# weiquan/salt

Hardware: AMD Instinct MI355X
Metric: Mreads/s aligned (100 bp SE, GRCh38+snp144) at 1/2/4/8 MI355X vs CPU ref (higher is better)
Workload: dtype u32; 1 GPU; GRCh38-scale synthetic (SURVEY 8d config 3 = BASELINE configs[2]): 3100000000 bp genome in 24 contigs, 14800000 SNPs, k=21, 1000000 x 100 bp SE reads per GPU per step, 8 distinct resident batches rotated, inputs and results resident in HBM; read_len=100, distinct_batches=8, options=default (-s 50 -m 1000, overlap = k), streams_per_gpu=4

## Files before the change

### salt_amd/csrc/salt_align.hip

```cpp
#include "salt_device.h"
#include "salt_kernels.h"

namespace salt {

#define WSYNC() do { __builtin_amdgcn_fence(__ATOMIC_ACQ_REL, "wavefront"); __builtin_amdgcn_wave_barrier(); \
                     __builtin_amdgcn_fence(__ATOMIC_ACQ_REL, "wavefront"); } while (0)

static constexpr int MAXL = SALT_MAX_READ_LEN;
static constexpr int SLOTS = SALT_MAX_SEED_SLOTS;
static constexpr int MAXLOC = SALT_MAX_LOCATE;
static constexpr int LVK = 31;
static_assert(offsetof(salt_result_t, strand) == 4 && offsetof(salt_result_t, mapq) == 7 && offsetof(salt_result_t, b0) == 8 &&
              offsetof(salt_result_t, b1) == 12 && offsetof(salt_result_t, seq_start) == 16 && offsetof(salt_result_t, seq_end) == 18 &&
              offsetof(salt_result_t, n_hits) == 20 && offsetof(salt_result_t, n_cigar) == 22 && offsetof(salt_result_t, skipped) == 23 &&
              offsetof(salt_result_t, hits) == 24 && sizeof(salt_hit_t) == 8, "salt_result_t header layout");
static constexpr int NHIT = 6;
__device__ __forceinline__ uint32_t mapq_quot(uint32_t x, uint32_t b0)
{
    const uint32_t v = 255u * x;
    return b0 == 1u ? v : b0 == 2u ? v / 2u : b0 == 3u ? v / 3u : v / b0;
}
static constexpr uint32_t INF = 255;

__device__ __forceinline__ uint32_t lane_id() { return threadIdx.x & 63u; }

typedef const uint32_t __attribute__((address_space(1))) *gp_u32;
typedef uint32_t u32x4_t __attribute__((ext_vector_type(4)));
typedef const u32x4_t __attribute__((address_space(1))) *gp_u32x4;
__device__ __forceinline__ gp_u32 as_global(const uint32_t *p) { return (gp_u32)p; }
__device__ __forceinline__ gp_u32x4 as_global(const uint4 *p) { return (gp_u32x4)(const void *)p; }

struct PhaseClock {
    unsigned long long *acc; uint64_t t;
    __device__ PhaseClock(unsigned long long *a) : acc(a), t(a ? __builtin_amdgcn_s_memtime() : 0) {}
    __device__ __forceinline__ void stamp(int slot)
    {
        if (!acc) return;
        uint64_t n = __builtin_amdgcn_s_memtime();
        if (lane_id() == 0) acc[slot] += (unsigned long long)(n - t);
        t = n;
    }
    __device__ __forceinline__ void add(int slot, unsigned long long v) { if (acc && lane_id() == 0) acc[slot] += v; }
};

__device__ __forceinline__ uint32_t read_base(const uint8_t *seq, uint32_t L, int strand, uint32_t i)
{
    if (strand == 0) return seq[i];
    uint32_t c = seq[L - 1 - i];
    return c < 4 ? 3 - c : c;
}

__device__ __forceinline__ uint32_t pk_nibbles(uint32_t x)
{
    uint32_t t = x & 0x0F0F0F0Fu;
    t = (t | (t >> 4)) & 0x00FF00FFu;
    return (t | (t >> 8)) & 0xFFFFu;
}

struct PackWords { uint32_t pm[64], tb[32], nm[16]; };

__global__ void __launch_bounds__(256)
k_pack(PackGeom pg, uint32_t n_reads, const uint8_t *__restrict__ seqs, const uint32_t *__restrict__ offs,
       uint32_t *__restrict__ pm, uint32_t *__restrict__ tb)
{
    extern __shared__ uint32_t pk_lds[];
    __shared__ uint32_t so[65];
    const uint32_t tpr = pg.nw32, rpb = 256 / tpr < 64 ? 256 / tpr : 64;
    const uint32_t wpr = pg.nw8 + pg.nw16 + pg.nw32;
    const uint32_t r0 = blockIdx.x * rpb, nr = n_reads - r0 < rpb ? n_reads - r0 : rpb;
    if (threadIdx.x <= nr) so[threadIdx.x] = offs[r0 + threadIdx.x];
    __syncthreads();
    const uint32_t cap = 8 * pg.nw8;
    const uint64_t total_bases = offs[n_reads];
    {
        const uint32_t rr = threadIdx.x / tpr, j = threadIdx.x - rr * tpr;
        if (rr < nr) {
            uint32_t L = so[rr + 1] - so[rr];
            if (L > cap) L = cap;
            const uintptr_t a0 = (uintptr_t)seqs + so[rr] + 32u * j, lo = (uintptr_t)seqs & ~(uintptr_t)3, hi = (uintptr_t)seqs + total_bases;
            const uintptr_t ab = a0 & ~(uintptr_t)3;
            const uint32_t sh = (uint32_t)(a0 & 3u) * 8u;
            uint32_t wv[9];
#pragma unroll
// ... 406 lines not shown
    const uint32_t tot_a = a1 - a0, tot = tot_a + (b1 - b0);
    const int i_top = (int)((uint32_t)sp.l_seed - ix.r_lkt_len) - 1;
    uint32_t n_aux = 0, n_sa = 0, n_text = 0, n_occ_c = 0, n_occ_r = 0;
    Walk w; w.ph = WK_IDLE; w.k = w.l = w.ext = w.p0 = 0; w.i = 0;
    SeedCtx c = seed_ctx_geom(sp, tb, 0, ix.r_lkt_len);
    uint32_t item = 0, cur = 0;
    bool is_r = false;
    const uint4 *qp = qa;
    for (;;) {
        const uint64_t idle = __ballot(w.ph == WK_IDLE);
        if (cur >= tot && idle == ~0ull) break;
        if (cur < tot) {
            const uint32_t t = cur + (uint32_t)__popcll(idle & lt);
            if (w.ph == WK_IDLE && t < tot) {
                const bool in_a = t < tot_a;
                qp = in_a ? qa + (size_t)t * WQ_REC : qb + (size_t)(t - tot_a) * WQ_REC; is_r = (in_a ? la : lb) == 0u; w.ph = WK_REC;
            }
            const uint32_t nx = cur + (uint32_t)__popcll(idle);
            cur = nx < tot ? nx : tot;
        }
        WalkReq q = walk_req_none();
        if (w.ph == WK_REC) { q.pa = qp; q.na = WQ_REC; }
        else if (w.ph != WK_IDLE) q = is_r ? seed_walk_issue<true>(ix, sp, c, w) : seed_walk_issue<false>(ix, sp, c, w);
        const WalkLoads ld = walk_fetch(q);
        bool done = false;
        uint4 row = make_uint4(1, 0, 0, 0);
        if (w.ph == WK_REC) {
            item = ld.a[0].x;
            c = seed_ctx_geom(sp, tb, item, ix.r_lkt_len);
            c.w0 = ld.a[1].x; c.w1 = ld.a[1].y; c.w2 = ld.a[1].z; c.n0 = ld.a[0].w; c.n1 = ld.a[1].w;
            done = is_r ? seed_walk_begin<true>(sp, c, ld.a[0].y, ld.a[0].z, i_top, w, row) : seed_walk_begin<false>(sp, c, ld.a[0].y, ld.a[0].z, i_top, w, row);
        } else if (w.ph != WK_IDLE) {
            done = is_r ? seed_walk_finish<true>(ix, sp, c, w, ld, row, n_occ_r, n_aux) : seed_walk_finish<false>(ix, sp, c, w, ld, row, n_occ_c, n_aux);
        }
        if (done && row.x <= row.y) { if (is_r) { row.w = sai_r_pack(sp.epoch, row.w); sai_r[item] = row; } else sai_c[item] = row; }
        n_sa += (n_aux >> 10) & 2047u; n_text += n_aux >> 21; n_aux = 0;
    }
    if (ctr) {
        for (int o = 32; o > 0; o >>= 1) { n_sa += __shfl_down(n_sa, o); n_text += __shfl_down(n_text, o); n_occ_c += __shfl_down(n_occ_c, o); n_occ_r += __shfl_down(n_occ_r, o); }
        if (lane_id() == 0) {
            atomicAdd(ctr + SALT_CTR_OCC_C, n_occ_c); atomicAdd(ctr + SALT_CTR_OCC_R, n_occ_r);
            atomicAdd(ctr + SALT_CTR_D_COCC_SEED, n_occ_c); atomicAdd(ctr + SALT_CTR_D_ROCC_SEED, n_occ_r);
            atomicAdd(ctr + SALT_CTR_D_SA_SEED, n_sa); atomicAdd(ctr + SALT_CTR_D_TEXT_SEED, n_text);
        }
    }
}

template <int NS> struct SaiListsT { uint32_t sp[2][NS], ep[2][NS], off[2][NS]; };
struct SaiLists { uint32_t *sp[2], *ep[2], *off[2]; };
template <int NS> __device__ __forceinline__ SaiLists sai_ref(SaiListsT<NS> &a) { return SaiLists{ { a.sp[0], a.sp[1] }, { a.ep[0], a.ep[1] }, { a.off[0], a.off[1] } }; }
struct LvTables { short L[LVK][64]; char A[LVK][64]; };
static constexpr int LLV_K = 12;
static constexpr int LLV_TW = 22;
static constexpr int LLV_W = 2 * LLV_K + 3;
static constexpr int LLV_N = 64;
struct LaneLv { uint32_t T[LLV_N * LLV_TW]; uint8_t rows[2][LLV_W][LLV_N]; };
struct LvBytes { uint8_t T[MAXL + 4 + 64]; uint8_t P[MAXL + 64]; };
template <int NS, bool LLV>
struct WaveLdsT {
    static constexpr bool HAS_LLV = LLV;
    static constexpr int N_SLOTS = NS;
    uint32_t pm[2][MAXL / 8];
    union U { SaiListsT<NS> sai; typename std::conditional<LLV, LaneLv, uint32_t>::type llv; LvBytes lvb; } u;
    uint8_t  cand_e[MAXLOC];
    uint32_t loci[MAXLOC];
    uint32_t hit_pos[2][NHIT];
    uint8_t  hit_nd[2][NHIT], hit_gap[2][NHIT];
    uint16_t cig[SALT_MAX_CIGAR_OPS];
    int      n_cig;
    alignas(8) uint8_t cargs[128];
};
typedef WaveLdsT<SLOTS, true> WaveLds;
typedef WaveLdsT<32, false> WaveLdsSmall;
typedef WaveLdsT<1, false> WaveLdsCigar;

struct Sai { uint32_t sp, ep, off; };
__device__ __forceinline__ Sai sai_get(const SaiLists &s, int w, int i) { return Sai{ s.sp[w][i], s.ep[w][i], s.off[w][i] }; }
__device__ __forceinline__ void sai_set(SaiLists &s, int w, int i, Sai v) { s.sp[w][i] = v.sp; s.ep[w][i] = v.ep; s.off[w][i] = v.off; }
__device__ __forceinline__ bool sai_ltv(Sai a, Sai b) { return a.ep - a.sp < b.ep - b.sp; }
__device__ __forceinline__ bool sai_lt(const SaiLists &s, int w, int i, int j) { return sai_ltv(sai_get(s, w, i), sai_get(s, w, j)); }
__device__ __forceinline__ void sai_swap(SaiLists &s, int w, int i, int j) { Sai a = sai_get(s, w, i), b = sai_get(s, w, j); sai_set(s, w, i, b); sai_set(s, w, j, a); }

__device__ void sai_insertsort(SaiLists &s, int w, int lo, int hi)
{
    for (int i = lo + 1; i < hi; ++i)
        for (int j = i; j > lo && sai_lt(s, w, j, j - 1); --j) sai_swap(s, w, j, j - 1);
}

__device__ void sai_combsort(SaiLists &s, int w, int base, int n)
{
    const double shrink = 1.2473309501039786540366528676643;
    int gap = n; bool do_swap;
    do {
        if (gap > 2) { gap = (int)(gap / shrink); if (gap == 9 || gap == 10) gap = 11; }
        do_swap = false;
        for (int i = 0; i < n - gap; ++i)
            if (sai_lt(s, w, base + i + gap, base + i)) { sai_swap(s, w, base + i, base + i + gap); do_swap = true; }
    } while (do_swap || gap > 2);
    if (gap != 1) sai_insertsort(s, w, base, base + n);
}

__device__ __attribute__((noinline)) void sai_introsort(SaiLists &s, int w, int n)
{
    if (n < 1) return;
    if (n == 2) { if (sai_lt(s, w, 1, 0)) sai_swap(s, w, 0, 1); return; }
    int d; for (d = 2; (1 << d) < n; ++d) { }
    d <<= 1;
    int st_l[24], st_r[24], st_d[24], top = 0;
    int lo = 0, hi = n - 1;
// ... 390 lines not shown
            }
        }
    }
}

__device__ __attribute__((noinline)) int lv_wave(const uint8_t *T, int tlen, const uint8_t *P, int plen, int k, LvTables *tab, int &d_fin)
{
    const int lane = (int)lane_id();
    const int d = lane - 31;
    const int ad = d < 0 ? -d : d;
    int Lprev = -2;
    const int end0 = plen < tlen ? plen : tlen;
    if (d == 0) { int i = 0; while (i < end0 && (P[i] & T[i]) != 0) ++i; Lprev = i; }
    const int r0 = __shfl(Lprev, 31);
    if (tab) tab->L[0][lane] = (short)Lprev;
    d_fin = 0;
    if (r0 == end0) return plen > end0 ? plen - end0 : 0;
    if (k > LVK - 1) k = LVK - 1;
    for (int e = 1; e <= k; ++e) {
        int left = __shfl_up(Lprev, 1), right = __shfl_down(Lprev, 1);
        if (lane == 0) left = -2;
        if (lane == 63) right = -2;
        const bool active = ad <= e && ad <= LVK - 1;
        int best = Lprev + 1; char act = 'X';
        if (left > best) { best = left; act = 'D'; }
        if (right + 1 > best) { best = right + 1; act = 'I'; }
        int cur = -2;
        if (active) {
            if (P[best] == T[d + best]) {
                int end = plen < tlen - d ? plen : tlen - d;
                if (best >= end) best = end;
                else { int i = best; while (i < end && (P[i] & T[d + i]) != 0) ++i; best = i; }
            }
            cur = best;
        }
        if (tab) { tab->L[e][lane] = (short)cur; tab->A[e][lane] = act; }
        uint64_t reach = __ballot(active && cur == plen);
        if (reach) {
            if (tab) {
                int rank = d == 0 ? 0 : (d < 0 ? 2 * ad - 1 : 2 * ad);
                int my = (active && cur == plen) ? rank : 1000;
                for (int o = 32; o > 0; o >>= 1) { int t = __shfl_xor(my, o); my = t < my ? t : my; }
                d_fin = my == 0 ? 0 : ((my & 1) ? -((my + 1) >> 1) : (my >> 1));
            }
            return e;
        }
        Lprev = cur;
    }
    return -1;
}

__device__ __attribute__((noinline)) uint32_t lv_lanes(LaneLv &s, const uint32_t *pm, int plen, int tlen, int k, bool active)
{
    const int lane = (int)lane_id() & (LLV_N - 1);
    const uint32_t *T = s.T + lane * LLV_TW;
    const int nwp = (plen + 7) >> 3;
    auto wP = [&](int i) -> uint32_t {
        const int j = i >> 3;
        const uint32_t lo = j < nwp ? pm[j] : 0u, hi = j + 1 < nwp ? pm[j + 1] : 0u;
        return __funnelshift_r(lo, hi, 4u * (uint32_t)(i & 7));
    };
    auto wT = [&](int i) -> uint32_t {
        if (i < 0) return i <= -8 ? 0u : T[0] << (4 * -i);
        const int j = i >> 3;
        const uint32_t lo = j < LLV_TW ? T[j] : 0u, hi = j + 1 < LLV_TW ? T[j + 1] : 0u;
        return __funnelshift_r(lo, hi, 4u * (uint32_t)(i & 7));
    };
    auto extend = [&](int d, int i, int end) -> int {
        while (i < end) {
            const uint32_t y = wP(i) & wT(d + i);
            const uint32_t z = ~(((y & 0x77777777u) + 0x77777777u) | y) & 0x88888888u;
            const int run = z ? (__ffs((int)z) - 1) >> 2 : 8;
            i += run;
            if (run < 8) break;
        }
        return i < end ? i : end;
    };
    auto RD = [&](int row, int d) -> int { return (int)s.rows[row][d + LLV_K + 1][lane] - 2; };
    auto WR = [&](int row, int d, int v) { s.rows[row][d + LLV_K + 1][lane] = (uint8_t)(v + 2); };
    for (int row = 0; row < 2; ++row) for (int d = 0; d < LLV_W; ++d) s.rows[row][d][lane] = 0;
    const int end0 = plen < tlen ? plen : tlen;
    uint32_t result = 255;
    bool done = !active;
    if (active) {
        const int i = extend(0, 0, end0);
        WR(0, 0, i);
        if (i == end0) { result = (uint32_t)(plen > end0 ? plen - end0 : 0); done = true; }
    }
    for (int e = 1; e <= k; ++e) {
        if (__ballot(!done) == 0) break;
        const int cur = e & 1, prev = cur ^ 1;
        for (int d = -e; d <= e; ++d) {
            if (done) continue;
            int best = RD(prev, d) + 1;
            const int left = RD(prev, d - 1), right = RD(prev, d + 1) + 1;
            if (left > best) best = left;
            if (right > best) best = right;
            if ((wP(best) & 15u) == (wT(d + best) & 15u)) {
                const int end = plen < tlen - d ? plen : tlen - d;
                best = best >= end ? end : extend(d, best, end);
            }
            if (best == plen) { result = (uint32_t)e; done = true; }
            else WR(cur, d, best);
        }
    }
    return result;
}

template <int VMAX, bool GAPF>
__device__ __forceinline__ void rule_unsorted(const uint32_t *pos, const uint8_t *val, const uint32_t n, const uint32_t L, const uint32_t ref_len,
                                              uint32_t &bound, bool &any, uint32_t &best_pos, uint32_t &best_v,
                                              uint32_t &n_hits, uint32_t &a0, uint32_t *hit_pos, uint8_t *hit_nd)
{
    const uint32_t lane = lane_id();
    const uint32_t NONE = 0xFFFFFFFFu;
    auto in_range = [&](uint32_t p) -> bool { return GAPF ? !(p + L + 4 >= ref_len) : p < ref_len; };
    uint32_t mp[VMAX + 1];
#pragma unroll
    for (int t = 0; t <= VMAX; ++t) mp[t] = NONE;
    uint32_t my_p = 0, my_v = NONE, n_p = 0;
    for (uint32_t b = 0; b < n; b += 64) {
        const uint32_t i = b + lane;
        uint32_t p = 0, v = NONE;
        if (i < n) { p = pos[i]; v = val[i]; }
        const bool in = i < n && v <= bound && in_range(p);
        if (in) {
#pragma unroll
            for (int t = 0; t <= VMAX; ++t) if (v == (uint32_t)t && p < mp[t]) mp[t] = p;
        }
        uint64_t m = __ballot(in);
        if (m && n_p <= 64u) {
            if (n_p + (uint32_t)__popcll(m) > 64u) n_p = 65u;
            else
                while (m) {
                    const int l = __ffsll((long long)m) - 1;
                    const uint32_t pl = (uint32_t)__builtin_amdgcn_readlane((int)p, l), vl = (uint32_t)__builtin_amdgcn_readlane((int)v, l);
                    if (lane == n_p) { my_p = pl; my_v = vl; }
                    ++n_p; m &= m - 1;
                }
        }
    }
#pragma unroll
    for (int t = 0; t <= VMAX; ++t)
        for (int o = 32; o > 0; o >>= 1) { const uint32_t x = (uint32_t)__shfl_xor((int)mp[t], o); mp[t] = x < mp[t] ? x : mp[t]; }
    uint32_t before[VMAX + 1];
    before[0] = NONE;
#pragma unroll
    for (int t = 1; t <= VMAX; ++t) before[t] = mp[t - 1] < before[t - 1] ? mp[t - 1] : before[t - 1];
    any = false; n_hits = 0;
#pragma unroll
    for (int t = VMAX; t >= 0; --t) if (mp[t] != NONE) { any = true; best_v = (uint32_t)t; best_pos = mp[t]; }
    if (!any) return;
    unsigned long long last = 0;
    const bool in_lanes = n_p <= 64u;
    unsigned long long my_key = ~0ull;
    if (in_lanes && lane < n_p) {
// ... 119 lines not shown
        w.u.lvb.P[i] = i < L ? (uint8_t)((w.pm[strand][i >> 3] >> (4 * (i & 7u))) & 15u) : (uint8_t)0;
    }
    WSYNC();
}

template <class W>
__device__ __attribute__((noinline)) void lv_cigar(const uint32_t *ref, W &w, LvTables *tabp, int strand, uint32_t L, uint32_t pos, int k)
{
    LvTables &tab = *tabp;
    lv_unpack(ref, w, strand, L, pos);
    int d_fin = 0;
    WSYNC();
    int e = lv_wave(w.u.lvb.T, (int)L + 4, w.u.lvb.P, (int)L, k, &tab, d_fin);
    __threadfence_block();
    WSYNC();
    if (lane_id() == 0) {
        int n = 0;
        uint16_t *cg = w.cig;
        if (e == 0) { cg[n++] = (uint16_t)((L << 4) | 0u); }
        else if (e > 0) {
            char act[LVK + 1]; int matched[LVK + 1];
            int cd = d_fin;
            for (int ce = e; ce >= 1; --ce) {
                char a = tab.A[ce][cd + 31];
                act[ce] = a;
                int cur = tab.L[ce][cd + 31];
                if (a == 'I') { matched[ce] = cur - tab.L[ce - 1][cd + 1 + 31] - 1; cd += 1; }
                else if (a == 'D') { matched[ce] = cur - tab.L[ce - 1][cd - 1 + 31]; cd -= 1; }
                else { matched[ce] = cur - tab.L[ce - 1][cd + 31] - 1; }
            }
            int acc = tab.L[0][31];
            int ce = 1;
            while (ce <= e) {
                char a = act[ce]; int cnt = 1;
                while (ce + 1 <= e && matched[ce] == 0 && act[ce + 1] == a) { ++cnt; ++ce; }
                if (a == 'X') acc += cnt;
                else {
                    if (acc != 0 && n < SALT_MAX_CIGAR_OPS) { cg[n++] = (uint16_t)((acc << 4) | 0); }
                    acc = 0;
                    if (n < SALT_MAX_CIGAR_OPS) cg[n++] = (uint16_t)((cnt << 4) | (a == 'I' ? 1 : 2));
                }
                if (matched[ce] > 0) acc += matched[ce];
                ++ce;
            }
            if (acc != 0 && n < SALT_MAX_CIGAR_OPS) cg[n++] = (uint16_t)((acc << 4) | 0);
        }
        w.n_cig = n;
    }
    WSYNC();
}

__device__ __forceinline__ void lane_text(const uint32_t *__restrict__ ref, uint32_t *T, uint32_t pos, uint32_t tl)
{
    const uint32_t w0 = pos >> 3, sh = (pos & 7u) * 4u, nwt = (tl + 7) >> 3;
    uint32_t wv[LLV_TW + 1];
#pragma unroll
    for (int j = 0; j <= LLV_TW; ++j) wv[j] = (uint32_t)j <= nwt ? ref[w0 + (uint32_t)j] : 0u;
#pragma unroll
    for (int j = 0; j < LLV_TW; ++j) {
        uint32_t word = 0;
        if ((uint32_t)j < nwt) {
            word = __funnelshift_r(wv[j], wv[j + 1], sh);
            const uint32_t rem = tl - (uint32_t)j * 8;
            if (rem < 8) word &= (1u << (4 * rem)) - 1u;
        }
        T[j] = word;
    }
}

__device__ __forceinline__ uint32_t store_gap_list(const uint32_t *loci, uint32_t n, uint32_t L, uint32_t ref_len, uint32_t *__restrict__ dst)
{
    const uint32_t lane = lane_id();
    const uint64_t lt = (1ull << lane) - 1ull;
    uint32_t n_out = 0;
    for (uint32_t b = 0; b < n; b += 64) {
        const uint32_t i = b + lane;
        const uint32_t pos = i < n ? loci[i] : 0u;
        const bool keep = i < n && !(pos + L + 4 >= ref_len);
        const uint64_t m = __ballot(keep);
        if (keep) dst[n_out + (uint32_t)__popcll(m & lt)] = pos;
        n_out += (uint32_t)__popcll(m);
    }
    return n_out;
}

template <bool PE, bool GL, class W>
__device__ __forceinline__ void align_general(const IndexView ix, const AlignParams ap, W &w, const uint32_t r,
                              const uint32_t *__restrict__ pm,
                              const uint4 *__restrict__ sai_c, const uint4 *__restrict__ sai_r,
                              salt_result_t *__restrict__ results, unsigned long long *__restrict__ ctr,
                              unsigned long long *phase, LvTables *lvtab, const GapBufs g, uint32_t *pe_loci, uint8_t *pe_cand)
{
    const uint32_t lane = lane_id();
    const uint64_t lt = (1ull << lane) - 1ull;
    const uint32_t *rec = pm + (uint64_t)r * ap.pg.pm_stride;
    const uint32_t L = rec[2 * ap.pg.nw8];
    salt_result_t *out = results + r;
    uint32_t c_sa_c = 0, c_sa_r = 0, c_verify = 0, c_vwords = 0, c_lv = 0, c_loci = 0, c_ctx_rej = 0, c_ctx_rows = 0;
    PhaseClock pc(phase);
    const uint64_t rt0 = phase ? __builtin_amdgcn_s_memrealtime() : 0;
    constexpr bool glob = GL;
    uint32_t *loci = glob ? pe_loci : w.loci;
    uint8_t *cand_e = glob ? pe_cand : w.cand_e;
    const uint32_t loci_cap = PE ? PE_LOCI_CAP : (uint32_t)MAXLOC;

    const uint32_t nw = (L + 7) >> 3;
    uint32_t n_amb = 0;
    for (uint32_t t = lane; t < 2 * nw; t += 64) {
        const uint32_t s = t >= nw, j = s ? t - nw : t;
        const uint32_t word = rec[s * ap.pg.nw8 + j];
        w.pm[s][j] = word;
        if (!s) n_amb += (uint32_t)__popc(word & (word >> 1) & (word >> 2) & (word >> 3) & 0x11111111u);
    }
    if (ap.max_amb < L) { for (int o = 32; o > 0; o >>= 1) n_amb += (uint32_t)__shfl_xor((int)n_amb, o); }
    else n_amb = 0;
    WSYNC();
    uint32_t q_pos = 0xFFFFFFFFu; uint32_t q_strand = 3, q_ndiff = 255, q_gap = 255;
    const bool too_short = L < (uint32_t)ap.l_seed;
    if (n_amb > ap.max_amb) {
        if (lane == 0) {
// ... 69 lines not shown
                    uint32_t o = 0;
                    if (lane == 0) o = atomicAdd(&g.gctl->pool_used, n);
                    o = (uint32_t)__shfl((int)o, 0);
                    ok = (uint64_t)o + n <= g.pool;
                    if (ok) for (uint32_t i = lane; i < n; i += 64) g.gloci[o + i] = loci[i];
                    ns[strand] = n; off[strand] = o;
                }
                const uint32_t ch0 = ok ? (ns[0] + LLV_N - 1) / LLV_N : 0, ch1 = ok ? (ns[1] + LLV_N - 1) / LLV_N : 0;
                uint32_t base = 0;
                if (ok && lane == 0) base = atomicAdd(&g.gctl->gap_items, ch0 + ch1);
                base = (uint32_t)__shfl((int)base, 0);
                ok = ok && (uint64_t)base + ch0 + ch1 <= g.items_cap;
                if (lane == 0) {
                    g.gq[slot] = ok ? r : 0xFFFFFFFFu;
                    g.gn[2 * slot] = ok ? ns[0] : 0; g.gn[2 * slot + 1] = ok ? ns[1] : 0;
                    g.goff[2 * slot] = off[0]; g.goff[2 * slot + 1] = off[1];
                }
                if (ok) {
                    for (uint32_t c = lane; c < ch0 + ch1; c += 64) g.gitems[base + c] = (slot << 11) | (c >= ch0 ? (0x400u | (c - ch0)) : c);
                    if (ctr) {
                        for (int o2 = 32; o2 > 0; o2 >>= 1) c_vwords += __shfl_down(c_vwords, o2);
                        if (lane == 0) {
                            atomicAdd(ctr + SALT_CTR_SA_C, c_sa_c); atomicAdd(ctr + SALT_CTR_SA_R, c_sa_r);
                            atomicAdd(ctr + SALT_CTR_VERIFY, c_verify); atomicAdd(ctr + SALT_CTR_VERIFY_WORDS, c_vwords);
                            atomicAdd(ctr + SALT_CTR_LV, ns[0] + ns[1]); atomicAdd(ctr + SALT_CTR_READS, 1ull);
                            atomicAdd(ctr + SALT_CTR_BASES, L); atomicAdd(ctr + SALT_CTR_LOCI, c_loci);
                            atomicAdd(ctr + SALT_CTR_D_SA_HEAVY, c_sa_c + c_sa_r);
                            atomicAdd(ctr + SALT_CTR_D_VERIFY_HEAVY, c_verify * (L <= 248 ? 4u : (((L + 7) >> 3) + 4u) / 4u));
                            atomicAdd(ctr + SALT_CTR_D_OUT_HEAVY, 5u * (ns[0] + ns[1]) + 16u);
                            if (ix.c_ctx) { atomicAdd(ctr + SALT_CTR_D_CTX_ROWS, c_ctx_rows); atomicAdd(ctr + SALT_CTR_D_CTX_REJECTED, c_ctx_rej); }
                        }
                    }
                    return;
                }
                WSYNC();
            }
        }
        if constexpr (!W::HAS_LLV) {
            if (lanes_fit && n_cand_nogap > 0) {
                if (lane == 0) g.ovq[atomicAdd(&g.gctl->ovq_count, 1u)] = r;
                return;
            }
        }
        for (int strand = 0; strand < 2; ++strand) {
            pc.stamp(SALT_CTR_T_GAP);
            const CandStats cs = build_candidates_call<PE, GL>(CandArgs{ ix.c_sa, ix.r_pos, sai_c, sai_r, ix.ref_len, ap.spr, ap.max_locate, r, L, strand, true, phase, pe_loci, loci_cap, ap.pe, true, ap.epoch, nullptr, nullptr, 0 }, w);
            if (glob) { loci = cs.in_lds ? w.loci : pe_loci; cand_e = cs.in_lds ? w.cand_e : pe_cand; }
            pc.t = phase ? __builtin_amdgcn_s_memtime() : 0;
            const uint32_t n_cand = cs.n_cand; c_sa_c += cs.n_sa_c; c_sa_r += cs.n_sa_r; c_loci += cs.n_loci;
            bool any = false;
            const bool lanes_ok = lanes_fit && W::HAS_LLV;
            if constexpr (W::HAS_LLV) if (lanes_ok) {
                const int k0 = gap_k0;
                for (uint32_t b = 0; b < n_cand; b += LLV_N) {
                    WSYNC();
                    const uint32_t i = b + lane;
                    bool act = false;
                    if (lane < LLV_N && i < n_cand) {
                        const uint32_t pos = loci[i];
                        act = !(pos > ix.ref_len || pos + L + 4 > ix.ref_len);
                        if (act) lane_text(ix.ref, w.u.llv.T + lane * LLV_TW, pos, L + 4);
                    }
                    const uint32_t e = lv_lanes(w.u.llv, w.pm[strand], (int)L, (int)L + 4, k0, act);
                    if (lane < LLV_N && i < n_cand) cand_e[i] = (uint8_t)e;
                }
                WSYNC();
            }
            for (uint32_t i = 0; i < n_cand; ++i) {
                uint32_t pos = loci[i];
                int e = -1;
                if (lanes_ok) { const uint32_t ev = cand_e[i]; e = (ev != 255 && (int)ev <= maxd) ? (int)ev : -1; }
                else if (!(pos > ix.ref_len || pos + L + 4 > ix.ref_len)) {
                    lv_unpack(ix.ref, w, strand, L, pos);
                    int dd;
                    e = lv_wave(w.u.lvb.T, (int)L + 4, w.u.lvb.P, (int)L, maxd, nullptr, dd);
                    WSYNC();
                }
                ++c_lv;
                if (e >= 0) {
                    if (e < maxd || !any) { maxd = e; q_gap = 1; q_ndiff = (uint32_t)e; q_strand = (uint32_t)strand; q_pos = pos; }
                    if (n_hits_s[strand] < NHIT && lane == 0) {
                        uint32_t h = n_hits_s[strand];
                        w.hit_pos[strand][h] = pos; w.hit_nd[strand][h] = (uint8_t)e; w.hit_gap[strand][h] = 1;
                    }
                    if (n_hits_s[strand] == 0) a0[strand] = (uint32_t)e;
                    if (n_hits_s[strand] < NHIT) ++n_hits_s[strand];
                    any = true;
                }
            }
            found[strand] = any;
            WSYNC();
        }
    }
    WSYNC();
    pc.stamp(SALT_CTR_T_GAP);

    int b0 = (int)q_ndiff, b1 = 100000, tot = 0;
    uint32_t nh[2] = { 0, 0 };
    uint32_t sel_idx[2][SALT_MAX_HITS];
    for (int s = 0; s < 2 && tot < ap.max_hits; ++s) {
        for (uint32_t j = 0; j < n_hits_s[s]; ++j) {
            uint32_t p = w.hit_pos[s][j];
            if (p == 0xFFFFFFFFu || p == q_pos) continue;
            if (a0[s] <= q_ndiff) {
                if ((int)a0[s] <= b1) b1 = (int)a0[s];
                if (nh[s] < SALT_MAX_HITS) sel_idx[s][nh[s]] = j;
                ++nh[s]; ++tot;
            }
            if (tot == ap.max_hits) break;
        }
    }
    uint32_t mapq = 0;
    if (b0 != 0) {
        uint32_t x = (uint32_t)(b0 > b1 ? b0 - b1 : b1 - b0);
        uint64_t q = mapq_quot(x, (uint32_t)b0);
        mapq = q < 254 ? (uint32_t)q : 254u;
// ... 72 lines not shown
    __shared__ W w;
    __shared__ uint32_t s_item;
    __shared__ unsigned long long s_phase[SALT_CTR_N];
    unsigned long long *phase = ctr ? s_phase : nullptr;
    if (ctr) { for (int i = threadIdx.x; i < SALT_CTR_N; i += 64) s_phase[i] = 0; }
    WSYNC();
    const uint32_t n_items = overflow_pass ? g.gctl->ovq_count : ap.all_heavy ? ap.n_reads : g.gctl->light_queued;
    uint32_t seg = blockIdx.x & (QUEUE_RANGES - 1u), tried = 0;
    for (;;) {
        if (threadIdx.x == 0) {
            uint32_t got = 0xFFFFFFFFu;
            if (overflow_pass) { got = atomicAdd(&g.gctl->ovq_head, 1u); if (got >= n_items) got = 0xFFFFFFFFu; }
            else got = pop_ranged(g.ranges, QueueRange::HEAVY, n_items, seg, tried);
            s_item = got;
        }
        WSYNC();
        const uint32_t it = s_item;
        WSYNC();
        if (it == 0xFFFFFFFFu) break;
        const uint32_t r = overflow_pass ? g.ovq[it] : ap.all_heavy ? it : queue[it];
        align_general<PE, GL>(ix, ap, w, r, pm, sai_c, sai_r, results, ctr, phase, lvtab + blockIdx.x, g,
                          pe_scr ? reinterpret_cast<uint32_t *>(pe_scr + (size_t)blockIdx.x * PE_LOCI_CAP * 5) : nullptr,
                          pe_scr ? pe_scr + (size_t)blockIdx.x * PE_LOCI_CAP * 5 + (size_t)PE_LOCI_CAP * 4 : nullptr);
        if (phase && threadIdx.x == 0) s_phase[SALT_CTR_HEAVY_READS] += 1;
        WSYNC();
    }
    if (phase) {
        WSYNC();
        for (int i = SALT_CTR_T_LOAD + (int)threadIdx.x; i < SALT_CTR_N; i += 64) if (s_phase[i]) atomicAdd(ctr + i, s_phase[i]);
    }
}

#ifndef SALT_HEAVY_WAVES
#define SALT_HEAVY_WAVES 4
#endif
#if SALT_HEAVY_WAVES > 0
#define HEAVY_OCC __attribute__((amdgpu_waves_per_eu(SALT_HEAVY_WAVES, SALT_HEAVY_WAVES)))
#else
#define HEAVY_OCC
#endif
#define HEAVY_KERNEL(NAME, PE, GL, LDS)                                                                                    \
__global__ void __launch_bounds__(64) HEAVY_OCC                                                                         \
NAME(IndexView ix, AlignParams ap, const uint32_t *__restrict__ pm,                                                     \
     const uint4 *__restrict__ sai_c, const uint4 *__restrict__ sai_r, salt_result_t *__restrict__ results,             \
     const uint32_t *__restrict__ queue, unsigned long long *__restrict__ ctr,                                          \
     LvTables *__restrict__ lvtab, GapBufs g, uint8_t *__restrict__ pe_scr, int overflow_pass)                          \
{ heavy_body<PE, GL, LDS>(ix, ap, pm, sai_c, sai_r, results, queue, ctr, lvtab, g, pe_scr, overflow_pass); }
HEAVY_KERNEL(k_heavy, false, false, WaveLdsSmall)
HEAVY_KERNEL(k_heavy_pe, true, true, WaveLdsSmall)
HEAVY_KERNEL(k_heavy_big, false, false, WaveLds)
HEAVY_KERNEL(k_heavy_pe_big, true, true, WaveLds)
HEAVY_KERNEL(k_heavy_glob, false, true, WaveLds)

struct GapLds { LaneLv llv; uint32_t pm[MAXL / 8]; };
__global__ void __launch_bounds__(64)
k_gap(IndexView ix, AlignParams ap, const uint32_t *__restrict__ pm, GapBufs g)
{
    __shared__ GapLds s;
    __shared__ uint32_t s_item;
    const uint32_t lane = lane_id();
    const uint32_t n_items = g.gctl->gap_items < g.items_cap ? g.gctl->gap_items : g.items_cap;
    uint32_t seg = blockIdx.x & (QUEUE_RANGES - 1u), tried = 0;
    for (;;) {
        if (threadIdx.x == 0) s_item = pop_ranged(g.ranges, QueueRange::GAP, n_items, seg, tried);
        WSYNC();
        const uint32_t it = s_item;
        WSYNC();
        if (it == 0xFFFFFFFFu) break;
        const uint32_t item = g.gitems[it], slot = item >> 11, strand = (item >> 10) & 1u, chunk = item & 1023u;
        const uint32_t r = g.gq[slot];
        const uint32_t *rec = pm + (uint64_t)r * ap.pg.pm_stride;
        const uint32_t L = rec[2 * ap.pg.nw8], nw = (L + 7) >> 3;
        for (uint32_t t = lane; t < nw; t += 64) s.pm[t] = rec[strand * ap.pg.nw8 + t];
        const uint32_t n = g.gn[2 * slot + strand], i = chunk * LLV_N + lane;
        const size_t row = g.goff[2 * slot + strand];
        bool act = false;
        if (lane < LLV_N && i < n) {
            const uint32_t pos = g.gloci[row + i];
            act = !(pos > ix.ref_len || pos + L + 4 > ix.ref_len);
            if (act) lane_text(ix.ref, s.llv.T + lane * LLV_TW, pos, L + 4);
        }
        WSYNC();
        const uint32_t e = lv_lanes(s.llv, s.pm, (int)L, (int)L + 4, ap.pe ? 3 : (int)(L / 10), act);
        if (lane < LLV_N && i < n) g.ge[row + i] = (uint8_t)e;
        WSYNC();
    }
}

struct FinLds { uint32_t hit_pos[2][NHIT]; uint8_t hit_nd[2][NHIT]; };
__global__ void __launch_bounds__(64)
k_gapfin(IndexView ix, AlignParams ap, const uint32_t *__restrict__ pm, salt_result_t *__restrict__ results, GapBufs g,
         unsigned long long *__restrict__ ctr)
{
    __shared__ FinLds w;
    __shared__ uint32_t s_item;
    const uint32_t lane = lane_id();
    const uint64_t lt = (1ull << lane) - 1ull;
    const uint32_t n_items = g.gctl->gap_slots < g.cap ? g.gctl->gap_slots : g.cap;
    uint32_t seg = blockIdx.x & (QUEUE_RANGES - 1u), tried = 0;
    for (;;) {
        if (threadIdx.x == 0) s_item = pop_ranged(g.ranges, QueueRange::GAPFIN, n_items, seg, tried);
        WSYNC();
        const uint32_t slot = s_item;
        WSYNC();
        if (slot == 0xFFFFFFFFu) break;
        const uint64_t rt0 = ctr ? __builtin_amdgcn_s_memrealtime() : 0;
        const uint32_t r = g.gq[slot];
        if (r == 0xFFFFFFFFu) continue;
        const uint32_t L = pm[(uint64_t)r * ap.pg.pm_stride + 2 * ap.pg.nw8];
        salt_result_t *out = results + r;
        uint32_t q_pos = 0xFFFFFFFFu, q_strand = 3, q_ndiff = 255, q_gap = 255;
        uint32_t bound = ap.pe ? 3u : L / 10;
        uint32_t n_hits_s[2] = { 0, 0 }, a0[2] = { 0, 0 };
        for (int strand = 0; strand < 2; ++strand) {
            const uint32_t n = g.gn[2 * slot + strand];
            const size_t row = g.goff[2 * slot + strand];
            bool any = false; uint32_t bp = 0, bv = 0;
            rule_unsorted<LLV_K, true>(g.gloci + row, g.ge + row, n, L, ix.ref_len, bound, any, bp, bv, n_hits_s[strand], a0[strand],
                                       w.hit_pos[strand], w.hit_nd[strand]);
            if (any) { q_pos = bp; q_ndiff = bv; q_gap = 1; q_strand = (uint32_t)strand; }
        }
        WSYNC();
        int b0 = (int)q_ndiff, b1 = 100000, tot = 0;
        uint32_t nh[2] = { 0, 0 };
        uint32_t sel_idx[2][SALT_MAX_HITS];
        for (int s = 0; s < 2 && tot < ap.max_hits; ++s)
            for (uint32_t j = 0; j < n_hits_s[s]; ++j) {
                const uint32_t p = w.hit_pos[s][j];
                if (p == 0xFFFFFFFFu || p == q_pos) continue;
                if (a0[s] <= q_ndiff) {
                    if ((int)a0[s] <= b1) b1 = (int)a0[s];
                    if (nh[s] < SALT_MAX_HITS) sel_idx[s][nh[s]] = j;
                    ++nh[s]; ++tot;
                }
                if (tot == ap.max_hits) break;
            }
// ... 624 lines not shown
{
    if (!ap.n_reads) return;
    static const bool no_half = getenv("SALT_GPU_NO_LIGHT2") && atoi(getenv("SALT_GPU_NO_LIGHT2"));
    if (!no_half && !ctr && !SALT_DIAG_VAL(ap.dbg_stop) && ap.spr <= (uint32_t)L2_SLOTS && ap.pg.nw8 <= 31) {
        static const int wv = getenv("SALT_GPU_L2_WAVES") ? atoi(getenv("SALT_GPU_L2_WAVES")) : 2;
        if (ap.pg.nw8 > 15) hipLaunchKernelGGL((k_light2<2, 8>), dim3((ap.n_reads + 3) / 4), dim3(128), 0, st, ix, ap, pm, sai_c, sai_r, results, qseg, ranges);
        else if (wv == 1) hipLaunchKernelGGL(k_light2<1>, dim3((ap.n_reads + 1) / 2), dim3(64), 0, st, ix, ap, pm, sai_c, sai_r, results, qseg, ranges);
        else hipLaunchKernelGGL(k_light2<2>, dim3((ap.n_reads + 3) / 4), dim3(128), 0, st, ix, ap, pm, sai_c, sai_r, results, qseg, ranges);
    } else
        hipLaunchKernelGGL(k_light, dim3((ap.n_reads + LT_WAVES - 1) / LT_WAVES), dim3(64 * LT_WAVES), 0, st, ix, ap, pm, sai_c, sai_r, results, qseg, ranges, ctr);
    hipLaunchKernelGGL(k_queue_pack, dim3(QUEUE_RANGES), dim3(256), 0, st, qseg, ranges, ap.n_reads, queue, ctl);
}
size_t queue_words(uint32_t max_reads) { return (size_t)max_reads * 2 + (size_t)QUEUE_RANGES * qseg_cap(max_reads); }

__global__ void __launch_bounds__(64)
k_diag_rule(uint32_t n_cases, const uint32_t *__restrict__ pos, const uint8_t *__restrict__ val, const uint32_t *__restrict__ offs,
            const uint32_t *__restrict__ bound_in, uint32_t L, uint32_t ref_len, int mode, uint32_t *__restrict__ out)
{
    __shared__ uint32_t hit_pos[NHIT];
    __shared__ uint8_t hit_nd[NHIT];
    const uint32_t c = blockIdx.x, lane = lane_id();
    if (c >= n_cases) return;
    const uint32_t o = offs[c], n = offs[c + 1] - o;
    uint32_t bound = bound_in[c], bp = 0, bv = 0, nh = 0, a0 = 0;
    bool any = false;
    if (lane < NHIT) { hit_pos[lane] = 0; hit_nd[lane] = 0; }
    WSYNC();
    if (mode == 0) rule_unsorted<3, false>(pos + o, val + o, n, L, ref_len, bound, any, bp, bv, nh, a0, hit_pos, hit_nd);
    else if (mode == 1) rule_sparse<3, false>(pos + o, val + o, n, L, ref_len, bound, any, bp, bv, nh, a0, hit_pos, hit_nd);
    else rule_unsorted<LLV_K, true>(pos + o, val + o, n, L, ref_len, bound, any, bp, bv, nh, a0, hit_pos, hit_nd);
    WSYNC();
    uint32_t *w = out + (size_t)c * (6 + 2 * NHIT);
    if (lane == 0) { w[0] = any; w[1] = any ? bp : 0; w[2] = any ? bv : 0; w[3] = nh; w[4] = nh ? a0 : 0; w[5] = bound; }
    if (lane < NHIT) { w[6 + 2 * lane] = lane < nh ? hit_pos[lane] : 0; w[7 + 2 * lane] = lane < nh ? hit_nd[lane] : 0; }
}

void launch_diag_rule(uint32_t n_cases, const uint32_t *pos, const uint8_t *val, const uint32_t *offs, const uint32_t *bound_in,
                      uint32_t L, uint32_t ref_len, int mode, uint32_t *out, hipStream_t st)
{
    if (n_cases) hipLaunchKernelGGL(k_diag_rule, dim3(n_cases), dim3(64), 0, st, n_cases, pos, val, offs, bound_in, L, ref_len, mode, out);
}
uint32_t diag_rule_words() { return 6 + 2 * NHIT; }

__host__ __device__ static inline bool lv_fit_dev(uint32_t L, uint32_t k) { return k <= (uint32_t)LLV_K && L + 4 <= 8u * (LLV_TW - 1); }
bool lv_lanes_fit(uint32_t L, uint32_t k) { return lv_fit_dev(L, k); }

__global__ void __launch_bounds__(64)
k_diag_lv(IndexView ix, uint32_t n_cases, const uint32_t *__restrict__ pos, const uint32_t *__restrict__ kdiff,
          const uint8_t *__restrict__ seqs, const uint32_t *__restrict__ offs, const uint32_t *__restrict__ lane_first,
          const uint32_t *__restrict__ lane_n, const uint32_t *__restrict__ lane_case, int32_t *__restrict__ out ,
          uint16_t *__restrict__ cig_out , LvTables *__restrict__ lvtab)
{
    __shared__ WaveLds w;
    __shared__ uint32_t lane_pm[LLV_N][LLV_TW];
    const uint32_t c = blockIdx.x, lane = lane_id();
    if (c >= n_cases) return;
    const uint32_t off = offs[c], L = offs[c + 1] - off, p = pos[c];
    const uint32_t nw = (L + 7) >> 3;
    auto pm_word = [&](uint32_t o, uint32_t j) -> uint32_t {
        uint32_t word = 0;
        for (uint32_t q = 0; q < 8; ++q) {
            uint32_t i = j * 8 + q, cc = i < L ? seqs[o + i] : 5u;
            word |= (cc < 4 ? (1u << cc) : (cc == 4 ? 15u : 0u)) << (4 * q);
        }
        return word;
    };
    for (uint32_t j = lane; j < nw; j += 64) w.pm[0][j] = pm_word(off, j);
    WSYNC();
    int32_t v = -2, e_wave = -1, n_cig = -2;
    if (p + L <= ix.ref_len) v = (int32_t)mismatch_capped(ix, w.pm[0], L, p);
    const bool in_range = !(p > ix.ref_len || p + L + 4 > ix.ref_len);
    const int k = (int)kdiff[c];
    if (in_range) {
        lv_unpack(ix.ref, w, 0, L, p);
        int dd;
        e_wave = lv_wave(w.u.lvb.T, (int)L + 4, w.u.lvb.P, (int)L, k, nullptr, dd);
        WSYNC();
    }
    const bool fit = lv_fit_dev(L, (uint32_t)k);
    const uint32_t gn = fit ? lane_n[c] : 0u;
    if (gn) {
        const uint32_t m = lane_case[lane_first[c] + lane % gn], mo = offs[m], mp = pos[m];
        for (uint32_t j = 0; j < nw; ++j) lane_pm[lane][j] = pm_word(mo, j);
        const bool act = !(mp > ix.ref_len || mp + L + 4 > ix.ref_len);
        if (act) lane_text(ix.ref, w.u.llv.T + lane * LLV_TW, mp, L + 4);
        WSYNC();
        const uint32_t el = lv_lanes(w.u.llv, lane_pm[lane], (int)L, (int)L + 4, k, act);
        if (lane < gn) out[(size_t)m * 4 + 2] = el == 255 ? -1 : (int32_t)el;
        WSYNC();
    }
    if (in_range && e_wave >= 0 && e_wave < LVK) {
        lv_cigar(ix.ref, w, lvtab + blockIdx.x, 0, L, p, e_wave);
        n_cig = w.n_cig;
        if (lane < (uint32_t)w.n_cig) cig_out[(size_t)c * SALT_MAX_CIGAR_OPS + lane] = w.cig[lane];
    }
    if (lane == 0) {
        out[(size_t)c * 4 + 0] = v; out[(size_t)c * 4 + 1] = e_wave; out[(size_t)c * 4 + 3] = n_cig;
        if (!fit) out[(size_t)c * 4 + 2] = -2;
    }
}

size_t lv_table_bytes() { return sizeof(LvTables); }

void launch_diag_lv(const IndexView &ix, uint32_t n, const uint32_t *pos, const uint32_t *kdiff, const uint8_t *seqs,
                    const uint32_t *offs, const uint32_t *lane_first, const uint32_t *lane_n, const uint32_t *lane_case,
                    int32_t *out, uint16_t *cig, void *lvtab, hipStream_t st)
{
    if (n) hipLaunchKernelGGL(k_diag_lv, dim3(n), dim3(64), 0, st, ix, n, pos, kdiff, seqs, offs, lane_first, lane_n, lane_case, out, cig,
                              static_cast<LvTables *>(lvtab));
}

__global__ void __launch_bounds__(64)
k_diag_verify(const uint32_t *__restrict__ ref, uint32_t ref_len, uint32_t n_cases, const uint8_t *__restrict__ seqs, const uint32_t *__restrict__ offs,
              const uint32_t *__restrict__ cand, const uint32_t *__restrict__ coffs, int mode, uint8_t *__restrict__ out)
{
    __shared__ uint32_t pm[64];
    __shared__ uint32_t loci[256];
    __shared__ uint8_t val[256];
    const uint32_t c = blockIdx.x, lane = lane_id();
    if (c >= n_cases) return;
    const uint32_t off = offs[c], L = offs[c + 1] - off, c0 = coffs[c];
    uint32_t n = coffs[c + 1] - c0;
    if (n > 256) n = 256;
    const uint32_t nw = (L + 7) >> 3;
    for (uint32_t j = lane; j < 64; j += 64) {
        uint32_t word = 0;
        for (uint32_t q = 0; q < 8 && j < nw; ++q) {
            const uint32_t i = j * 8 + q, cc = i < L ? seqs[off + i] : 5u;
            word |= (cc < 4 ? (1u << cc) : (cc == 4 ? 15u : 0u)) << (4 * q);
        }
        pm[j] = word;
    }
    for (uint32_t i = lane; i < n; i += 64) { loci[i] = cand[c0 + i]; val[i] = 77; }
    WSYNC();
    IndexView ix; ix.ref = ref; ix.ref_len = ref_len;
    if (mode == 0) { for (uint32_t i = lane; i < n; i += 64) val[i] = (uint8_t)mismatch_capped(ix, pm, L, loci[i]); }
    else if (mode == 1) verify_quads<8>(ref, ref_len, pm, L, loci, n, val);
    else if (mode == 2) verify_quads<8, 8>(ref, ref_len, pm, L, loci, n, val);
// ... 168 lines not shown
```

Baseline: 480.5 Mreads/s.

## Keep lane-parallel Landau-Vishkin diagonals in registers and transpose text in LDS

Rewrites the per-lane Landau-Vishkin kernel so the diagonal rows live in a fully unrolled register array instead of per-lane byte rows in LDS. Each lane's text words are now stored interleaved (word-major, lane-minor) so LDS accesses across a wave hit different banks. Pattern words are copied into a zero-padded shared buffer so fetches need no bounds checks. This removes LDS traffic and bank conflicts in the inner loop, at the cost of more VGPRs and a fixed unrolled loop over all 25 diagonals regardless of e.

Result: faster. 514.8 Mreads/s, median of 6 (+7.1%).

```diff
diff --git a/salt_amd/csrc/salt_align.hip b/salt_amd/csrc/salt_align.hip
--- a/salt_amd/csrc/salt_align.hip
+++ b/salt_amd/csrc/salt_align.hip
@@ -29,6 +29,8 @@
 typedef const u32x4_t __attribute__((address_space(1))) *gp_u32x4;
 __device__ __forceinline__ gp_u32 as_global(const uint32_t *p) { return (gp_u32)p; }
 __device__ __forceinline__ gp_u32x4 as_global(const uint4 *p) { return (gp_u32x4)(const void *)p; }
+typedef const uint32_t __attribute__((address_space(3))) *lds_u32;
+__device__ __forceinline__ lds_u32 as_lds(const uint32_t *p) { return (lds_u32)p; }
 
 struct PhaseClock {
     unsigned long long *acc; uint64_t t;
@@ -541,9 +543,13 @@
 struct LvTables { short L[LVK][64]; char A[LVK][64]; };
 static constexpr int LLV_K = 12;
 static constexpr int LLV_TW = 22;
-static constexpr int LLV_W = 2 * LLV_K + 3;
 static constexpr int LLV_N = 64;
-struct LaneLv { uint32_t T[LLV_N * LLV_TW]; uint8_t rows[2][LLV_W][LLV_N]; };
+static constexpr int LLV_WIN = 4;
+static constexpr int LLV_TS = LLV_TW + 2;
+static constexpr int LLV_PW = LLV_TW;
+static_assert(((8 * (LLV_TW - 1) - LLV_WIN + LLV_K) >> 3) + 2 <= LLV_TS, "text words of the longest window at the widest bound");
+static_assert(((8 * (LLV_TW - 1) - LLV_WIN) >> 3) + 2 <= LLV_PW, "pattern words of the longest read");
+struct LaneLv { uint32_t T[LLV_TS * LLV_N]; uint32_t P[LLV_PW]; };
 struct LvBytes { uint8_t T[MAXL + 4 + 64]; uint8_t P[MAXL + 64]; };
 template <int NS, bool LLV>
 struct WaveLdsT {
@@ -1040,56 +1046,57 @@
 
 __device__ __attribute__((noinline)) uint32_t lv_lanes(LaneLv &s, const uint32_t *pm, int plen, int tlen, int k, bool active)
 {
+    constexpr int LLV_W = 2 * LLV_K + 1;
     const int lane = (int)lane_id() & (LLV_N - 1);
-    const uint32_t *T = s.T + lane * LLV_TW;
-    const int nwp = (plen + 7) >> 3;
-    auto wP = [&](int i) -> uint32_t {
-        const int j = i >> 3;
-        const uint32_t lo = j < nwp ? pm[j] : 0u, hi = j + 1 < nwp ? pm[j + 1] : 0u;
-        return __funnelshift_r(lo, hi, 4u * (uint32_t)(i & 7));
+    const lds_u32 T = as_lds(s.T) + lane, P = as_lds(pm);
+    auto fetch = [&](int i, int t, uint32_t &p, uint32_t &x) {
+        const lds_u32 pp = P + (i >> 3), tt = T + (t >> 3) * LLV_N;
+        const uint32_t p0 = pp[0], p1 = pp[1], t0 = tt[0], t1 = tt[LLV_N];
+        p = __funnelshift_r(p0, p1, 4u * (uint32_t)(i & 7));
+        x = __funnelshift_r(t0, t1, 4u * (uint32_t)(t & 7));
     };
-    auto wT = [&](int i) -> uint32_t {
-        if (i < 0) return i <= -8 ? 0u : T[0] << (4 * -i);
-        const int j = i >> 3;
-        const uint32_t lo = j < LLV_TW ? T[j] : 0u, hi = j + 1 < LLV_TW ? T[j + 1] : 0u;
-        return __funnelshift_r(lo, hi, 4u * (uint32_t)(i & 7));
+    auto run_of = [](uint32_t p, uint32_t x) -> int {
+        const uint32_t y = p & x;
+        const uint32_t z = ~(((y & 0x77777777u) + 0x77777777u) | y) & 0x88888888u;
+        return z ? __builtin_ctz(z) >> 2 : 8;
     };
-    auto extend = [&](int d, int i, int end) -> int {
-        while (i < end) {
-            const uint32_t y = wP(i) & wT(d + i);
-            const uint32_t z = ~(((y & 0x77777777u) + 0x77777777u) | y) & 0x88888888u;
-            const int run = z ? (__ffs((int)z) - 1) >> 2 : 8;
-            i += run;
-            if (run < 8) break;
-        }
-        return i < end ? i : end;
+    auto reach = [&](int d, int best, bool gated) -> int {
+        uint32_t p, x;
+        fetch(best, d + best, p, x);
+        const int end = plen < tlen - d ? plen : tlen - d;
+        const bool open = !gated || ((p ^ x) & 15u) == 0;
+        int run = run_of(p, x), i = best + run;
+        if (open && run == 8) while (i < end) { fetch(i, d + i, p, x); run = run_of(p, x); i += run; if (run < 8) break; }
+        i = i < end ? i : end;
+        return open ? i : best;
     };
-    auto RD = [&](int row, int d) -> int { return (int)s.rows[row][d + LLV_K + 1][lane] - 2; };
-    auto WR = [&](int row, int d, int v) { s.rows[row][d + LLV_K + 1][lane] = (uint8_t)(v + 2); };
-    for (int row = 0; row < 2; ++row) for (int d = 0; d < LLV_W; ++d) s.rows[row][d][lane] = 0;
+    int row[LLV_W];
+#pragma unroll
+    for (int j = 0; j < LLV_W; ++j) row[j] = -2;
     const int end0 = plen < tlen ? plen : tlen;
     uint32_t result = 255;
     bool done = !active;
     if (active) {
-        const int i = extend(0, 0, end0);
-        WR(0, 0, i);
+        const int i = reach(0, 0, false);
+        row[LLV_K] = i;
         if (i == end0) { result = (uint32_t)(plen > end0 ? plen - end0 : 0); done = true; }
     }
     for (int e = 1; e <= k; ++e) {
         if (__ballot(!done) == 0) break;
-        const int cur = e & 1, prev = cur ^ 1;
-        for (int d = -e; d <= e; ++d) {
-            if (done) continue;
-            int best = RD(prev, d) + 1;
-            const int left = RD(prev, d - 1), right = RD(prev, d + 1) + 1;
-            if (left > best) best = left;
-            if (right > best) best = right;
-            if ((wP(best) & 15u) == (wT(d + best) & 15u)) {
-                const int end = plen < tlen - d ? plen : tlen - d;
-                best = best >= end ? end : extend(d, best, end);
-            }
-            if (best == plen) { result = (uint32_t)e; done = true; }
-            else WR(cur, d, best);
+        int carry = -2;
+#pragma unroll
+        for (int d = -LLV_K; d <= LLV_K; ++d) {
+            if ((d < 0 ? -d : d) > e) continue;
+            const int mid = row[d + LLV_K], right = d < LLV_K ? row[d + LLV_K + 1] : -2;
+            int best = mid + 1;
+            if (carry > best) best = carry;
+            if (right + 1 > best) best = right + 1;
+            carry = mid;
+            if (!done) {
+                best = reach(d, best, true);
+                if (best == plen) { result = (uint32_t)e; done = true; }
+                else row[d + LLV_K] = best;
+            }
         }
     }
     return result;
@@ -1315,7 +1322,7 @@
 
 __device__ __forceinline__ void lane_text(const uint32_t *__restrict__ ref, uint32_t *T, uint32_t pos, uint32_t tl)
 {
-    const uint32_t w0 = pos >> 3, sh = (pos & 7u) * 4u, nwt = (tl + 7) >> 3;
+    const uint32_t w0 = pos >> 3, sh = (pos & 7u) * 4u, nwt = (tl + 7) >> 3, nst = ((tl - LLV_WIN + LLV_K) >> 3) + 2;
     uint32_t wv[LLV_TW + 1];
 #pragma unroll
     for (int j = 0; j <= LLV_TW; ++j) wv[j] = (uint32_t)j <= nwt ? ref[w0 + (uint32_t)j] : 0u;
@@ -1327,8 +1334,15 @@
             const uint32_t rem = tl - (uint32_t)j * 8;
             if (rem < 8) word &= (1u << (4 * rem)) - 1u;
         }
-        T[j] = word;
-    }
+        if ((uint32_t)j < nst) T[j * LLV_N] = word;
+    }
+#pragma unroll
+    for (int j = LLV_TW; j < LLV_TS; ++j) if ((uint32_t)j < nst) T[j * LLV_N] = 0u;
+}
+template <class F>
+__device__ __forceinline__ void lane_pattern(uint32_t *P, uint32_t nw, uint32_t first, uint32_t step, F word)
+{
+    for (uint32_t j = first; j < (uint32_t)LLV_PW; j += step) P[j] = j < nw ? word(j) : 0u;
 }
 
 __device__ __forceinline__ uint32_t store_gap_list(const uint32_t *loci, uint32_t n, uint32_t L, uint32_t ref_len, uint32_t *__restrict__ dst)
@@ -1504,6 +1518,8 @@
             const bool lanes_ok = lanes_fit && W::HAS_LLV;
             if constexpr (W::HAS_LLV) if (lanes_ok) {
                 const int k0 = gap_k0;
+                WSYNC();
+                lane_pattern(w.u.llv.P, (L + 7) >> 3, lane, 64u, [&](uint32_t j) { return w.pm[strand][j]; });
                 for (uint32_t b = 0; b < n_cand; b += LLV_N) {
                     WSYNC();
                     const uint32_t i = b + lane;
@@ -1511,9 +1527,9 @@
                     if (lane < LLV_N && i < n_cand) {
                         const uint32_t pos = loci[i];
                         act = !(pos > ix.ref_len || pos + L + 4 > ix.ref_len);
-                        if (act) lane_text(ix.ref, w.u.llv.T + lane * LLV_TW, pos, L + 4);
+                        if (act) lane_text(ix.ref, w.u.llv.T + lane, pos, L + 4);
                     }
-                    const uint32_t e = lv_lanes(w.u.llv, w.pm[strand], (int)L, (int)L + 4, k0, act);
+                    const uint32_t e = lv_lanes(w.u.llv, w.u.llv.P, (int)L, (int)L + 4, k0, act);
                     if (lane < LLV_N && i < n_cand) cand_e[i] = (uint8_t)e;
                 }
                 WSYNC();
@@ -1692,11 +1708,10 @@
 HEAVY_KERNEL(k_heavy_pe_big, true, true, WaveLds)
 HEAVY_KERNEL(k_heavy_glob, false, true, WaveLds)
 
-struct GapLds { LaneLv llv; uint32_t pm[MAXL / 8]; };
 __global__ void __launch_bounds__(64)
 k_gap(IndexView ix, AlignParams ap, const uint32_t *__restrict__ pm, GapBufs g)
 {
-    __shared__ GapLds s;
+    __shared__ LaneLv s;
     __shared__ uint32_t s_item;
     const uint32_t lane = lane_id();
     const uint32_t n_items = g.gctl->gap_items < g.items_cap ? g.gctl->gap_items : g.items_cap;
@@ -1711,17 +1726,17 @@
         const uint32_t r = g.gq[slot];
         const uint32_t *rec = pm + (uint64_t)r * ap.pg.pm_stride;
         const uint32_t L = rec[2 * ap.pg.nw8], nw = (L + 7) >> 3;
-        for (uint32_t t = lane; t < nw; t += 64) s.pm[t] = rec[strand * ap.pg.nw8 + t];
+        lane_pattern(s.P, nw, lane, 64u, [&](uint32_t j) { return rec[strand * ap.pg.nw8 + j]; });
         const uint32_t n = g.gn[2 * slot + strand], i = chunk * LLV_N + lane;
         const size_t row = g.goff[2 * slot + strand];
         bool act = false;
         if (lane < LLV_N && i < n) {
             const uint32_t pos = g.gloci[row + i];
             act = !(pos > ix.ref_len || pos + L + 4 > ix.ref_len);
-            if (act) lane_text(ix.ref, s.llv.T + lane * LLV_TW, pos, L + 4);
+            if (act) lane_text(ix.ref, s.T + lane, pos, L + 4);
         }
         WSYNC();
-        const uint32_t e = lv_lanes(s.llv, s.pm, (int)L, (int)L + 4, ap.pe ? 3 : (int)(L / 10), act);
+        const uint32_t e = lv_lanes(s, s.P, (int)L, (int)L + 4, ap.pe ? 3 : (int)(L / 10), act);
         if (lane < LLV_N && i < n) g.ge[row + i] = (uint8_t)e;
         WSYNC();
     }
@@ -2452,7 +2467,7 @@
           uint16_t *__restrict__ cig_out , LvTables *__restrict__ lvtab)
 {
     __shared__ WaveLds w;
-    __shared__ uint32_t lane_pm[LLV_N][LLV_TW];
+    __shared__ uint32_t lane_pm[LLV_N][LLV_PW];
     const uint32_t c = blockIdx.x, lane = lane_id();
     if (c >= n_cases) return;
     const uint32_t off = offs[c], L = offs[c + 1] - off, p = pos[c];
@@ -2481,9 +2496,9 @@
     const uint32_t gn = fit ? lane_n[c] : 0u;
     if (gn) {
         const uint32_t m = lane_case[lane_first[c] + lane % gn], mo = offs[m], mp = pos[m];
-        for (uint32_t j = 0; j < nw; ++j) lane_pm[lane][j] = pm_word(mo, j);
+        lane_pattern(lane_pm[lane], nw, 0u, 1u, [&](uint32_t j) { return pm_word(mo, j); });
         const bool act = !(mp > ix.ref_len || mp + L + 4 > ix.ref_len);
-        if (act) lane_text(ix.ref, w.u.llv.T + lane * LLV_TW, mp, L + 4);
+        if (act) lane_text(ix.ref, w.u.llv.T + lane, mp, L + 4);
         WSYNC();
         const uint32_t el = lv_lanes(w.u.llv, lane_pm[lane], (int)L, (int)L + 4, k, act);
         if (lane < gn) out[(size_t)m * 4 + 2] = el == 255 ? -1 : (int32_t)el;
```
